# s22s/erased-cells

Measured on AMD Instinct MI355X. Metric: Gcells/s + HBM-GB/s roofline %, u8/u16->f64 16384^2, 1/2/4/8 GPUs, higher is better.
Workload: dtype f64

## Files before the change

erased-cells_amd/csrc/ec_binop_kernels.hpp:

```cpp
#pragma once

#include "ec_device.hpp"

namespace ecd {

constexpr int kBlock = 256;
constexpr int kWave = 64;
constexpr int kWavesPerBlock = kBlock / kWave;

template <bool NT, typename V>
__device__ __forceinline__ V load_vec(const V* p) {
    if constexpr (NT) return nt_load(p);
    else return plain_load(p);
}

__device__ __forceinline__ size_t two_front_tile() {
    const size_t b = blockIdx.x;
    return (b & 1) ? size_t(gridDim.x) - 1 - (b >> 1) : (b >> 1);
}

template <typename L, typename R, int OP, int U>
__device__ __forceinline__ void binop_direct_tile(const L* __restrict__ l, const R* __restrict__ r,
                                                  double* __restrict__ out, size_t npairs, size_t tile, unsigned cacheable) {
    using D2 = vec<double, 2>;
    constexpr bool FP = is_fp<L>::value || is_fp<R>::value;
    constexpr bool SM = is_small_int<L>::value && is_small_int<R>::value;
    constexpr size_t TILE = size_t(kBlock) * U;
    D2* __restrict__ op = reinterpret_cast<D2*>(out);
    const size_t base = tile * TILE + threadIdx.x;
    if (tile * TILE + TILE <= npairs) {
        cells<L, 2> a[U];
        cells<R, 2> b[U];
        policy_arms<2>(cacheable, [&](auto bits) {
            constexpr unsigned B = decltype(bits)::value;
#pragma unroll
            for (int j = 0; j < U; ++j) {
                a[j] = load_cells<!(B & 1u), L, 2>(l + 2 * (base + size_t(j) * kBlock));
                b[j] = load_cells<!(B & 2u), R, 2>(r + 2 * (base + size_t(j) * kBlock));
            }
        });
        if constexpr (OP == EC_DIV && SM && !FP) {
#pragma unroll
            for (int j = 0; j < U; ++j) {
                double av[2], bv[2], q[2], y[2], e[2];
                bool zero = false;
#pragma unroll
                for (int k = 0; k < 2; ++k) {
                    av[k] = to_f64(a[j][k]);
                    bv[k] = to_f64(b[j][k]);
                    zero = zero || b[j][k] == 0;
                }
                div_small_int_nonzero_staged<2>(av, bv, q, y, e);
                if (__builtin_expect(__builtin_amdgcn_ballot_w64(zero) != 0, 0)) {
#pragma unroll
                    for (int i = 0; i < 2; ++i) q[i] = bv[i] == 0.0 ? div_by_zero(av[i]) : q[i];
                }
                nt_store(D2{q[0], q[1]}, op + base + size_t(j) * kBlock);
            }
        } else {
#pragma unroll
            for (int j = 0; j < U; ++j) {
                const double av[2] = {to_f64(a[j][0]), to_f64(a[j][1])}, bv[2] = {to_f64(b[j][0]), to_f64(b[j][1])};
                double o[2];
                cell_op_n<OP, FP, SM, 2>(av, bv, o);
                nt_store(D2{o[0], o[1]}, op + base + size_t(j) * kBlock);
            }
        }
    } else {
#pragma unroll
        for (int j = 0; j < U; ++j) {
            const size_t p = base + size_t(j) * kBlock;
            if (p < npairs) {
                const cells<L, 2> a = load_cells<true, L, 2>(l + 2 * p);
                const cells<R, 2> b = load_cells<true, R, 2>(r + 2 * p);
                D2 o;
                o.x = cell_op<OP, FP, SM>(to_f64(a[0]), to_f64(b[0]));
                o.y = cell_op<OP, FP, SM>(to_f64(a[1]), to_f64(b[1]));
                nt_store(o, op + p);
            }
        }
    }
}

template <typename L, typename R, int OP, int U>
__device__ __forceinline__ void binop_direct_body(const L* __restrict__ l, const R* __restrict__ r,
                                                  double* __restrict__ out, size_t n, unsigned head_and_policy) {
    constexpr bool FP = is_fp<L>::value || is_fp<R>::value;
    constexpr bool SM = is_small_int<L>::value && is_small_int<R>::value;
    const unsigned head = head_and_policy & 0xffu, cacheable = head_and_policy >> 8;
    if (head) {
        if (blockIdx.x == 0 && threadIdx.x < head)
            st_cell(cell_op<OP, FP, SM>(to_f64(ld_cell(l + threadIdx.x)), to_f64(ld_cell(r + threadIdx.x))), out + threadIdx.x);
        l += head;
        r += head;
        out += head;
        n -= head;
    }
    binop_direct_tile<L, R, OP, U>(l, r, out, n >> 1, two_front_tile(), cacheable);
    if ((n & 1) && blockIdx.x == 0 && threadIdx.x == 0)
        st_cell(cell_op<OP, FP, SM>(to_f64(ld_cell(l + n - 1)), to_f64(ld_cell(r + n - 1))), out + n - 1);
}

template <typename L, int OP, int U, bool NANRULE = true>
__device__ __forceinline__ void binop_scalar_tile(const L* __restrict__ l, double s, double* __restrict__ out,
                                                  size_t npairs, size_t tile, unsigned cacheable) {
    using D2 = vec<double, 2>;
    constexpr bool FP = NANRULE;
    constexpr size_t TILE = size_t(kBlock) * U;
    D2* __restrict__ op = reinterpret_cast<D2*>(out);
    const size_t base = tile * TILE + threadIdx.x;
    if (tile * TILE + TILE <= npairs) {
        cells<L, 2> a[U];
        policy_arms<1>(cacheable, [&](auto bits) {
            constexpr unsigned B = decltype(bits)::value;
#pragma unroll
            for (int j = 0; j < U; ++j) a[j] = load_cells<!(B & 1u), L, 2>(l + 2 * (base + size_t(j) * kBlock));
        });
#pragma unroll
        for (int j = 0; j < U; ++j) {
            const double av[2] = {to_f64(a[j][0]), to_f64(a[j][1])}, bv[2] = {s, s};
            double o[2];
            cell_op_n<OP, FP, false, 2>(av, bv, o);
            nt_store(D2{o[0], o[1]}, op + base + size_t(j) * kBlock);
        }
    } else {
#pragma unroll
        for (int j = 0; j < U; ++j) {
            const size_t p = base + size_t(j) * kBlock;
            if (p < npairs) {
                const cells<L, 2> a = load_cells<true, L, 2>(l + 2 * p);
                D2 o;
                o.x = cell_op<OP, FP>(to_f64(a[0]), s);
                o.y = cell_op<OP, FP>(to_f64(a[1]), s);
                nt_store(o, op + p);
            }
        }
    }
}

template <typename L, int OP, int U, bool NANRULE = true>
__global__ __launch_bounds__(kBlock) void k_binop_scalar_direct(const L* __restrict__ l, double s,
                                                                double* __restrict__ out, size_t n, unsigned head_and_policy) {
    const unsigned head = head_and_policy & 0xffu, cacheable = head_and_policy >> 8;
    if (head) {
        if (blockIdx.x == 0 && threadIdx.x < head) st_cell(cell_op<OP, true>(to_f64(ld_cell(l + threadIdx.x)), s), out + threadIdx.x);
        l += head;
        out += head;
        n -= head;
    }
    binop_scalar_tile<L, OP, U, NANRULE>(l, s, out, n >> 1, two_front_tile(), cacheable);
    if ((n & 1) && blockIdx.x == 0 && threadIdx.x == 0) st_cell(cell_op<OP, true>(to_f64(ld_cell(l + n - 1)), s), out + n - 1);
}

template <typename L, typename R, int OP>
__global__ __launch_bounds__(kBlock) void k_binop_cellwise(const L* __restrict__ l, const R* __restrict__ r,
                                                           double* __restrict__ out, size_t n) {
    constexpr bool FP = is_fp<L>::value || is_fp<R>::value;
    constexpr bool SM = is_small_int<L>::value && is_small_int<R>::value;
    const size_t stride = size_t(gridDim.x) * kBlock;
    for (size_t i = size_t(blockIdx.x) * kBlock + threadIdx.x; i < n; i += stride)
        out[i] = cell_op<OP, FP, SM>(to_f64(l[i]), to_f64(r[i]));
}

template <typename L, int OP>
__global__ __launch_bounds__(kBlock) void k_binop_scalar_cellwise(const L* __restrict__ l, double s,
                                                                  double* __restrict__ out, size_t n) {
    const size_t stride = size_t(gridDim.x) * kBlock;
    for (size_t i = size_t(blockIdx.x) * kBlock + threadIdx.x; i < n; i += stride)
        out[i] = cell_op<OP, true>(to_f64(l[i]), s);
}

constexpr int kLdsChunks = 2;
constexpr size_t kLdsWaveCells = 128 * kLdsChunks;

template <typename T>
struct Staged {
    static constexpr bool value = sizeof(T) <= 4;
    using Load = vec<uint32_t, int(sizeof(T))>;
    static constexpr int kSlabBytes = value ? int(kLdsWaveCells * sizeof(T)) : 16;
};

using u32x4 = vec<uint32_t, 4>;

template <typename L, typename R, int OP>
__device__ __forceinline__ void binop_lds_body(const L* __restrict__ l, const R* __restrict__ r,
                                               double* __restrict__ out, size_t n) {
    using L2 = vec<L, 2>;
    using R2 = vec<R, 2>;
    using D2 = vec<double, 2>;
    constexpr bool FP = is_fp<L>::value || is_fp<R>::value;
    constexpr bool SM = is_small_int<L>::value && is_small_int<R>::value;
    constexpr bool SL = Staged<L>::value, SR = Staged<R>::value;

    __shared__ __attribute__((aligned(16))) unsigned char slab_l[kWavesPerBlock][Staged<L>::kSlabBytes];
    __shared__ __attribute__((aligned(16))) unsigned char slab_r[kWavesPerBlock][Staged<R>::kSlabBytes];

    const int lane = threadIdx.x & (kWave - 1);
    const int wave = threadIdx.x / kWave;
    const size_t nfull = n / kLdsWaveCells;
    const size_t t = two_front_tile() * kWavesPerBlock + wave;
    if (t < nfull) {
        const size_t cell0 = t * kLdsWaveCells;
        L2 a[kLdsChunks];
        R2 b[kLdsChunks];
        typename Staged<L>::Load sl{};
        typename Staged<R>::Load sr{};
        if constexpr (SL) {
            sl = nt_load(reinterpret_cast<const typename Staged<L>::Load*>(l + cell0) + lane);
        } else {
#pragma unroll
            for (int j = 0; j < kLdsChunks; ++j) a[j] = nt_load(reinterpret_cast<const L2*>(l + cell0) + j * kWave + lane);
        }
        if constexpr (SR) {
            sr = nt_load(reinterpret_cast<const typename Staged<R>::Load*>(r + cell0) + lane);
        } else {
#pragma unroll
            for (int j = 0; j < kLdsChunks; ++j) b[j] = nt_load(reinterpret_cast<const R2*>(r + cell0) + j * kWave + lane);
        }
        if constexpr (SL) reinterpret_cast<typename Staged<L>::Load*>(slab_l[wave])[lane] = sl;
        if constexpr (SR) reinterpret_cast<typename Staged<R>::Load*>(slab_r[wave])[lane] = sr;
        if constexpr (SL || SR) {
            __builtin_amdgcn_fence(__ATOMIC_RELEASE, "wavefront");
            __builtin_amdgcn_wave_barrier();
            __builtin_amdgcn_fence(__ATOMIC_ACQUIRE, "wavefront");
        }
        if constexpr (SL) {
#pragma unroll
            for (int j = 0; j < kLdsChunks; ++j) a[j] = reinterpret_cast<const L2*>(slab_l[wave])[j * kWave + lane];
        }
        if constexpr (SR) {
#pragma unroll
            for (int j = 0; j < kLdsChunks; ++j) b[j] = reinterpret_cast<const R2*>(slab_r[wave])[j * kWave + lane];
        }
        D2* o2 = reinterpret_cast<D2*>(out + cell0);
#pragma unroll
        for (int j = 0; j < kLdsChunks; ++j) {
            const double av[2] = {to_f64(a[j].x), to_f64(a[j].y)}, bv[2] = {to_f64(b[j].x), to_f64(b[j].y)};
            double o[2];
            cell_op_n<OP, FP, SM, 2>(av, bv, o);
            nt_store(D2{o[0], o[1]}, o2 + j * kWave + lane);
        }
    }
    if (blockIdx.x == 0)
        for (size_t i = nfull * kLdsWaveCells + threadIdx.x; i < n; i += kBlock)
            st_cell(cell_op<OP, FP, SM>(to_f64(ld_cell(l + i)), to_f64(ld_cell(r + i))), out + i);
}

template <typename L, typename R, int OP, int U>
__global__ __launch_bounds__(kBlock) void k_binop_direct(const L* __restrict__ l, const R* __restrict__ r,
                                                         double* __restrict__ out, size_t n, unsigned head = 0) {
    binop_direct_body<L, R, OP, U>(l, r, out, n, head);
}

template <typename L, typename R, int OP>
__global__ __launch_bounds__(kBlock) void k_binop_lds(const L* __restrict__ l, const R* __restrict__ r,
                                                      double* __restrict__ out, size_t n) {
    binop_lds_body<L, R, OP>(l, r, out, n);
}

__device__ __forceinline__ void mask_and_body(const uint8_t* __restrict__ lm, const uint8_t* __restrict__ rm,
                                              uint8_t* __restrict__ om, size_t n, unsigned cacheable) {
    const size_t ngroups = n / 16;
    const u32x4* __restrict__ a = reinterpret_cast<const u32x4*>(lm);
    const u32x4* __restrict__ b = reinterpret_cast<const u32x4*>(rm);
    u32x4* __restrict__ o = reinterpret_cast<u32x4*>(om);
    const size_t stride = size_t(gridDim.x) * kBlock;
    for (size_t g = size_t(blockIdx.x) * kBlock + threadIdx.x; g < ngroups; g += stride) {
        u32x4 x, y;
        policy_arms<2>(cacheable >> 2, [&](auto bits) {
            constexpr unsigned B = decltype(bits)::value;
            x = load_vec<!(B & 1u)>(a + g);
            y = load_vec<!(B & 2u)>(b + g);
        });
        mask_store(x & y, o + g);
    }
    if (blockIdx.x == 0)
        for (size_t i = ngroups * 16 + threadIdx.x; i < n; i += kBlock) st_cell<uint8_t>(ld_cell(lm + i) & ld_cell(rm + i), om + i);
}

template <typename L, typename R, int OP, int U, bool LDS>
__global__ __launch_bounds__(kBlock) void k_masked_binop(const L* __restrict__ l, const uint8_t* __restrict__ lm,
                                                         const R* __restrict__ r, const uint8_t* __restrict__ rm,
                                                         double* __restrict__ out, uint8_t* __restrict__ om, size_t n,
                                                         unsigned head) {
    if constexpr (LDS) binop_lds_body<L, R, OP>(l, r, out, n);
    else binop_direct_body<L, R, OP, U>(l, r, out, n, head);
    mask_and_body(lm, rm, om, n, head >> 8);
}

template <typename L, typename R, int OP>
__global__ __launch_bounds__(kBlock) void k_masked_binop_cellwise(const L* __restrict__ l, const uint8_t* __restrict__ lm,
                                                                  const R* __restrict__ r, const uint8_t* __restrict__ rm,
                                                                  double* __restrict__ out, uint8_t* __restrict__ om, size_t n) {
    constexpr bool FP = is_fp<L>::value || is_fp<R>::value;
    constexpr bool SM = is_small_int<L>::value && is_small_int<R>::value;
    const size_t stride = size_t(gridDim.x) * kBlock;
    for (size_t i = size_t(blockIdx.x) * kBlock + threadIdx.x; i < n; i += stride) {
        out[i] = cell_op<OP, FP, SM>(to_f64(l[i]), to_f64(r[i]));
        om[i] = lm[i] & rm[i];
    }
}

}
```

erased-cells_amd/csrc/ec_binop_tu.hpp:

```cpp
#pragma once

#include <hip/hip_runtime.h>

#include <cmath>

#include "ec_binop_kernels.hpp"
#include "ec_runtime.hpp"

namespace ecd {

static inline unsigned lds_cap(int knob, int rule_kb) { return static_cast<unsigned>(knob >= 0 ? knob : rule_kb) << 10; }

template <typename L, typename R, int OP>
static ec_status launch_binop_pair(const void* l, const void* r, size_t n, double* out, hipStream_t s) {
    const Tuning& tu = tuning();
    const L* lp = static_cast<const L*>(l);
    const R* rp = static_cast<const R*>(r);
    constexpr int U = kBinopU;
    if (!aligned16(l, r, out)) {
        k_binop_cellwise<L, R, OP><<<grid_capped((n + kBlock - 1) / kBlock, 8), kBlock, 0, s>>>(lp, rp, out, n);
        return check_launch("binop(cellwise)");
    }
    constexpr bool kCanStage = Staged<L>::value || Staged<R>::value;
    const int variant = tu.binop_variant.load();
    const size_t stream_bytes[2] = {n * sizeof(L), l == r ? 0 : n * sizeof(R)};
    unsigned policy = cache_plan(stream_bytes, 2, n * sizeof(double));
    if (l == r && (policy & 1u)) policy |= 2u;
    constexpr bool kRulePair = kCanStage && ((sizeof(L) == 8) != (sizeof(R) == 8)) && (sizeof(L) <= 4 || sizeof(R) <= 4);
    const bool by_rule = variant < 0 && kRulePair && policy == 0 && n >= (size_t(1) << 20);
    if (kCanStage && (variant == 1 || by_rule)) {
        const size_t tiles = (n / kLdsWaveCells + kWavesPerBlock - 1) / kWavesPerBlock;
        constexpr unsigned kStatic = kWavesPerBlock * unsigned(Staged<L>::kSlabBytes + Staged<R>::kSlabBytes);
        const int knob = tu.binop_lds_kb.load();
        const unsigned lds = knob >= 0 ? unsigned(knob) << 10 : by_rule ? 32000u - kStatic : 0u;
        k_binop_lds<L, R, OP><<<grid_for(tiles), kBlock, lds, s>>>(lp, rp, out, n);
        if (by_rule) lds_rule_launches().fetch_add(1, std::memory_order_relaxed);
        return check_launch(by_rule ? "binop(lds, by rule)" : "binop(lds)");
    }
    const LoadedStream st[2] = {{l, sizeof(L)}, {r, sizeof(R)}};
    const unsigned head = peel_head(st, 2, n);
    const size_t tiles = (((n - head) >> 1) + size_t(kBlock) * U - 1) / (size_t(kBlock) * U);
    k_binop_direct<L, R, OP, U><<<grid_for(tiles), kBlock, lds_cap(tuning().binop_lds_kb.load(), sizeof(L) == 8 && sizeof(R) == 8 ? 48 : 0), s>>>(lp, rp, out, n, head | (policy << 8));
    return check_launch("binop(direct)");
}

template <typename L, typename R, int OP>
static ec_status launch_masked_pair(const void* l, const uint8_t* lm, const void* r, const uint8_t* rm, size_t n,
                                    double* out, uint8_t* om, hipStream_t s) {
    const Tuning& tu = tuning();
    const L* lp = static_cast<const L*>(l);
    const R* rp = static_cast<const R*>(r);
    constexpr int U = kBinopU;
    if (!aligned16(l, r, out) || !aligned16(lm, rm, om)) {
        k_masked_binop_cellwise<L, R, OP><<<grid_capped((n + kBlock - 1) / kBlock, 8), kBlock, 0, s>>>(lp, lm, rp, rm, out, om, n);
        return check_launch("masked_binop(cellwise)");
    }
    constexpr bool kCanStage = Staged<L>::value || Staged<R>::value;
    if (kCanStage && tu.binop_variant == 1) {
        const size_t tiles = (n / kLdsWaveCells + kWavesPerBlock - 1) / kWavesPerBlock;
        k_masked_binop<L, R, OP, U, true><<<grid_for(tiles), kBlock, lds_cap(tu.binop_lds_kb.load(), 0), s>>>(lp, lm, rp, rm, out, om, n, 0u);
        return check_launch("masked_binop(lds)");
    }
    const LoadedStream st[2] = {{l, sizeof(L)}, {r, sizeof(R)}};
    const unsigned head = peel_head(st, 2, n);
    const size_t tiles = (((n - head) >> 1) + size_t(kBlock) * U - 1) / (size_t(kBlock) * U);
    const size_t stream_bytes[4] = {n * sizeof(L), l == r ? 0 : n * sizeof(R), n, lm == rm ? 0 : n};
    unsigned policy = cache_plan(stream_bytes, 4, n * sizeof(double));
    if (l == r && (policy & 1u)) policy |= 2u;
    if (lm == rm && (policy & 4u)) policy |= 8u;
    k_masked_binop<L, R, OP, U, false><<<grid_for(tiles), kBlock, 0, s>>>(lp, lm, rp, rm, out, om, n, head | (policy << 8));
    return check_launch("masked_binop(direct)");
}


template <typename L, int OP>
static ec_status launch_scalar(const void* l, double rhs, size_t n, double* out, hipStream_t s) {
    const L* lp = static_cast<const L*>(l);
    constexpr int U = kBinopU;
    if (!aligned16(l, out, out)) {
        k_binop_scalar_cellwise<L, OP><<<grid_capped((n + kBlock - 1) / kBlock, 8), kBlock, 0, s>>>(lp, rhs, out, n);
        return check_launch("binop_scalar(cellwise)");
    }
    const LoadedStream st[1] = {{l, sizeof(L)}};
    const unsigned head = peel_head(st, 1, n);
    const size_t tiles = (((n - head) >> 1) + size_t(kBlock) * U - 1) / (size_t(kBlock) * U);
    const size_t stream_bytes[1] = {n * sizeof(L)};
    const unsigned policy = cache_plan(stream_bytes, 1, n * sizeof(double));
    const unsigned lds = lds_cap(tuning().scalar_lds_kb.load(), sizeof(L) == 8 ? 32 : 0);
    if constexpr (!is_fp<L>::value) {
        if (std::isfinite(rhs) && !(OP == EC_DIV && rhs == 0.0)) {
            k_binop_scalar_direct<L, OP, U, false><<<grid_for(tiles), kBlock, lds, s>>>(lp, rhs, out, n, head | (policy << 8));
            return check_launch("binop_scalar(direct, no NaN possible)");
        }
    }
    k_binop_scalar_direct<L, OP, U><<<grid_for(tiles), kBlock, lds, s>>>(lp, rhs, out, n, head | (policy << 8));
    return check_launch("binop_scalar(direct)");
}

template <int OP>
ec_status dispatch_binop(int lt, const void* l, int rt, const void* r, size_t n, double* out, hipStream_t s) {
#define EC_ROW(LID, LT)                                                                         \
    case LID:                                                                                   \
        switch (rt) {                                                                           \
            case EC_U8: return launch_binop_pair<LT, uint8_t, OP>(l, r, n, out, s);             \
            case EC_U16: return launch_binop_pair<LT, uint16_t, OP>(l, r, n, out, s);           \
            case EC_U32: return launch_binop_pair<LT, uint32_t, OP>(l, r, n, out, s);           \
            case EC_U64: return launch_binop_pair<LT, uint64_t, OP>(l, r, n, out, s);           \
            case EC_I8: return launch_binop_pair<LT, int8_t, OP>(l, r, n, out, s);              \
            case EC_I16: return launch_binop_pair<LT, int16_t, OP>(l, r, n, out, s);            \
            case EC_I32: return launch_binop_pair<LT, int32_t, OP>(l, r, n, out, s);            \
            case EC_I64: return launch_binop_pair<LT, int64_t, OP>(l, r, n, out, s);            \
            case EC_F32: return launch_binop_pair<LT, float, OP>(l, r, n, out, s);              \
            case EC_F64: return launch_binop_pair<LT, double, OP>(l, r, n, out, s);             \
        }                                                                                       \
        break;
    switch (lt) { EC_WITH_CT(EC_ROW) }
#undef EC_ROW
    return set_error(EC_ERR_UNSUPPORTED_TYPE, "binop: bad dtype");
// ... 44 lines not shown
```

erased-cells_amd/csrc/ec_expr_jit.hip:

```cpp
#include <dlfcn.h>
#include <hip/hip_runtime.h>

#include <atomic>
#include <condition_variable>
#include <cstdlib>
#include <cstring>
#include <algorithm>
#include <deque>
#include <iterator>
#include <limits>
#include <map>
#include <memory>
#include <mutex>
#include <string>
#include <thread>
#include <unordered_map>
#include <vector>

#include "ec_expr_jit.hpp"
#include "ec_lattice.hpp"
#include "ec_runtime.hpp"

namespace ecd {

namespace {

const char* const kPrelude = R"SRC(
typedef double D2 __attribute__((ext_vector_type(2)));
typedef unsigned int U2 __attribute__((ext_vector_type(2)));
typedef unsigned int U4 __attribute__((ext_vector_type(4)));
typedef unsigned short W1 __attribute__((aligned(1)));
typedef unsigned int W2 __attribute__((aligned(1)));
typedef U2 W4 __attribute__((aligned(1)));
typedef U4 W8 __attribute__((aligned(1)));
typedef D2 DO __attribute__((aligned(1)));
typedef unsigned long long u64;
// the result's 16-byte store: write-through and non-temporal, as the library's own value stores (ec_device.hpp stream_store_asm;
// `s_nop 1`: a VALU write of the data registers needs two wait states behind a store of more than 64 bits)
static __device__ __forceinline__ void st16(D2 v, DO* p) { asm volatile("global_store_dwordx4 %0, %1, off sc1 nt\n\ts_nop 1" ::"v"(p), "v"(v)); }
#define FOR _Pragma("unroll") for (int i = 0; i < N; ++i)
// cv_bin_op! on NaN (ec_device.hpp cell_op<OP, true>): the first NaN operand, quieted; the x86 default NaN when neither is one
static __device__ __forceinline__ double fixnan(double t, double a, double b) {
    const u64 f = (a != a) ? (__builtin_bit_cast(u64, a) | 0x0008000000000000ull)
                : (b != b) ? (__builtin_bit_cast(u64, b) | 0x0008000000000000ull) : 0xFFF8000000000000ull;
    return (t != t) ? __builtin_bit_cast(double, f) : t;
}
// The quotient of two integers of magnitude ≤ 131070 held as f64 (≤ 16-bit cells, their sums and differences): v_rcp_f64, one
// Newton step, the quotient, its exact residual and one correction — ec_device.hpp div_small_int, proven against the IEEE
// expansion on that whole square (tools/div_small_check.hip); b == 0 gives what the f64 divide gives: ±inf, the x86 default
// NaN for 0/0 (an integer-derived zero is +0).
static __device__ __forceinline__ double divs(double a, double b) {
    double y = __builtin_amdgcn_rcp(b);
    const double e = __builtin_fma(-b, y, 1.0);
    y = __builtin_fma(y, e, y);
    double q = a * y;
    const double r = __builtin_fma(-b, q, a);
    q = __builtin_fma(r, y, q);
    const double z = a == 0.0 ? __builtin_bit_cast(double, 0xFFF8000000000000ull) : (a > 0.0 ? __builtin_inf() : -__builtin_inf());
    return b == 0.0 ? z : q;
}
// tested once per pair of cells (v_cmp_u_f64 r0, r1 is true when either is NaN), handled out of line, wave-uniform branch
#define NANFIX(A, B)                                                                                  \
    {                                                                                                 \
        bool nan = false;                                                                             \
        _Pragma("unroll") for (int i = 0; i + 1 < N; i += 2) nan = nan || __builtin_isunordered(t[i], t[i + 1]); \
        if (N & 1) nan = nan || (t[N - 1] != t[N - 1]);                                               \
        if (__builtin_expect(__builtin_amdgcn_ballot_w64(nan) != 0, 0)) { FOR t[i] = fixnan(t[i], A, B); } \
    }
)SRC";

const char* const kCellType[10] = {"unsigned char", "unsigned short", "unsigned int", "unsigned long long", "signed char",
                                   "short",         "int",            "long long",    "float",              "double"};

// ... 124 lines not shown
             "        if (__builtin_amdgcn_ballot_w64(special) == 0) {\n"
             "            _Pragma(\"unroll\") for (int i = 0; i < NC; ++i) {\n"
             "                fmin = __builtin_fmin(fmin, valid[i] ? o[i] : fmin);\n                fmax = __builtin_fmax(fmax, valid[i] ? o[i] : fmax);\n            }\n"
             "        } else {\n"
             "            _Pragma(\"unroll\") for (int i = 0; i < NC; ++i)\n                if (valid[i]) {\n"
             "                    const long long k = okey(o[i]);\n                    a = ~k > a ? ~k : a;\n                    b = k > b ? k : b;\n                }\n"
             "        }\n"
             "    }\n"
             "    {\n        const long long k0 = okey(fmin), k1 = okey(fmax);\n        a = ~k0 > a ? ~k0 : a;\n        b = k1 > b ? k1 : b;\n    }\n"
             "    if (blockIdx.x == 0 && threadIdx.x < 2) {  // the peeled head cell (lane 0) and the odd tail cell (lane 1)\n"
             "        const bool do_it = threadIdx.x == 0 ? head != 0 : ((n - head) & 1) != 0;\n"
             "        const unsigned long i = threadIdx.x == 0 ? 0 : n - 1;\n"
             "        if (do_it) {\n";
        for (int k2 = 0; k2 < 4; ++k2) {
            const std::string K = std::to_string(k2);
            o += "            const double a" + K + "[1] = {" + (k2 < ns ? "cell" + K + "(p" + K + ", i)" : std::string("0.0")) + "};\n";
        }
        o += "            double q[1];\n            run<1>(a0, a1, a2, a3, c0, c1, c2, c3, c4, c5, c6, c7, q);\n            bool ok = true;\n";
        for (int k2 = 0; k2 < ea.nmask; ++k2)
            o += "            ok = ok && __builtin_nontemporal_load((const unsigned char*)m" + std::to_string(k2) + " + i) != 0;\n";
        o += "            if (ok) {\n                const long long k = okey(q[0]);\n                a = ~k > a ? ~k : a;\n                b = k > b ? k : b;\n            }\n"
             "        }\n    }\n"
             "    __shared__ long long sa[256], sb[256];\n"
             "    sa[threadIdx.x] = a;\n    sb[threadIdx.x] = b;\n    __syncthreads();\n"
             "    for (int w = 128; w > 0; w >>= 1) {\n"
             "        if ((int)threadIdx.x < w) {\n"
             "            sa[threadIdx.x] = sa[threadIdx.x + w] > sa[threadIdx.x] ? sa[threadIdx.x + w] : sa[threadIdx.x];\n"
             "            sb[threadIdx.x] = sb[threadIdx.x + w] > sb[threadIdx.x] ? sb[threadIdx.x + w] : sb[threadIdx.x];\n"
             "        }\n        __syncthreads();\n    }\n"
             "    if (threadIdx.x == 0) {\n"
             "        __hip_atomic_fetch_max(keys2, sa[0], __ATOMIC_RELAXED, __HIP_MEMORY_SCOPE_AGENT);\n"
             "        __hip_atomic_fetch_max(keys2 + 1, sb[0], __ATOMIC_RELAXED, __HIP_MEMORY_SCOPE_AGENT);\n"
             "    }\n}\n";
        return o;
    }
    o += "extern \"C\" __global__ __launch_bounds__(256) void ec_expr_jit(const char* p0, const char* p1, const char* p2, const char* p3, ";
    o += scal;
    o += ", double* __restrict__ out, unsigned long n, unsigned head, const char* m0, const char* m1, const char* m2, const char* m3, "
         "unsigned char* __restrict__ out_mask) {\n"
         "    constexpr int U = 2, NC = 2 * U;\n"
         "    const unsigned long npairs = (n - head) >> 1, TILE = 256ul * U;\n"
         "    const unsigned long blk = blockIdx.x, tile = (blk & 1) ? (unsigned long)gridDim.x - 1 - (blk >> 1) : (blk >> 1);  // two fronts\n"
         "    const unsigned long base = tile * TILE + threadIdx.x;\n"
         "    DO* op = (DO*)(out + head);\n"
         "    double s0[NC] = {}, s1[NC] = {}, s2[NC] = {}, s3[NC] = {}, o[NC];\n";
    for (int k = 0; k < ns; ++k)
        o += "    const char* b" + std::to_string(k) + " = p" + std::to_string(k) + " + (unsigned long)head * " + std::to_string(ecl::size_of(ea.dt[k])) + ";\n";
    o += "    const bool full = tile * TILE + TILE <= npairs;\n"
         "    if (full) {\n        _Pragma(\"unroll\") for (int j = 0; j < U; ++j) {\n            const unsigned long pr = base + j * 256ul;\n";
    for (int k = 0; k < ns; ++k) {
        const std::string K = std::to_string(k);
        o += "            ld" + K + "(b" + K + ", pr, s" + K + "[2 * j], s" + K + "[2 * j + 1]);\n";
    }
    o += "        }\n    } else {\n        _Pragma(\"unroll\") for (int j = 0; j < U; ++j) {\n            const unsigned long pr = base + j * 256ul;\n            if (pr < npairs) {\n";
    for (int k = 0; k < ns; ++k) {
        const std::string K = std::to_string(k);
        o += "                ld" + K + "(b" + K + ", pr, s" + K + "[2 * j], s" + K + "[2 * j + 1]);\n";
    }
    o += "            }\n        }\n    }\n"
         "    run<NC>(s0, s1, s2, s3, c0, c1, c2, c3, c4, c5, c6, c7, o);\n"
         "    _Pragma(\"unroll\") for (int j = 0; j < U; ++j) {\n        const unsigned long pr = base + j * 256ul;\n"
         "        if (full || pr < npairs) st16(D2{o[2 * j], o[2 * j + 1]}, op + pr);\n    }\n"
         "    if (blockIdx.x == 0 && threadIdx.x < 2) {  // the peeled head cell (lane 0) and the odd tail cell (lane 1)\n"
         "        const bool do_it = threadIdx.x == 0 ? head != 0 : ((n - head) & 1) != 0;\n"
         "        const unsigned long i = threadIdx.x == 0 ? 0 : n - 1;\n"
         "        if (do_it) {\n";
    for (int k = 0; k < 4; ++k) {
        const std::string K = std::to_string(k);
        o += "            const double a" + K + "[1] = {" + (k < ns ? "cell" + K + "(p" + K + ", i)" : std::string("0.0")) + "};\n";
    }
    o += "            double q[1];\n            run<1>(a0, a1, a2, a3, c0, c1, c2, c3, c4, c5, c6, c7, q);\n"
         "            __builtin_nontemporal_store(q[0], out + i);\n        }\n    }\n";
    if (ea.nmask > 0) {
        o += "    {\n        const unsigned long ngroups = n / 16, stride = (unsigned long)gridDim.x * 256ul;\n"
             "        for (unsigned long g = (unsigned long)blockIdx.x * 256ul + threadIdx.x; g < ngroups; g += stride) {\n"
             "            U4 acc = {0xffffffffu, 0xffffffffu, 0xffffffffu, 0xffffffffu};\n";
        for (int k = 0; k < ea.nmask; ++k) {
            const bool nt = !((ea.cacheable >> (4 + k)) & 1u);
            o += std::string("            acc &= ") + (nt ? "__builtin_nontemporal_load(" : "*(") + "(const W8*)m" + std::to_string(k) + " + g);\n";
        }
        o += "            __builtin_nontemporal_store(acc, (W8*)out_mask + g);\n        }\n"
             "        if (blockIdx.x == 0)\n            for (unsigned long i = ngroups * 16 + threadIdx.x; i < n; i += 256ul) {\n"
             "                unsigned char acc = __builtin_nontemporal_load((const unsigned char*)m0 + i);\n";
        for (int k = 1; k < ea.nmask; ++k)
            o += "                acc &= __builtin_nontemporal_load((const unsigned char*)m" + std::to_string(k) + " + i);\n";
        o += "                __builtin_nontemporal_store(acc, out_mask + i);\n            }\n    }\n";
    }
    o += "}\n";
    return o;
}

namespace {

struct Hiprtc {
    int (*create)(void** prog, const char* src, const char* name, int nh, const char** headers, const char** names) = nullptr;
    int (*compile)(void* prog, int nopt, const char** opts) = nullptr;
    int (*code_size)(void* prog, size_t* n) = nullptr;
    int (*code)(void* prog, char* out) = nullptr;
    int (*log_size)(void* prog, size_t* n) = nullptr;
    int (*log)(void* prog, char* out) = nullptr;
    int (*destroy)(void** prog) = nullptr;
    const char* (*error_string)(int) = nullptr;
    std::string load_error;
};

Hiprtc g_rtc;
std::once_flag g_rtc_once;

void load_hiprtc() {
    void* h = nullptr;
    if (const char* named = std::getenv("EC_HIPRTC_LIB")) {
        h = dlopen(named, RTLD_NOW | RTLD_LOCAL);
    } else {
        for (const char* name : {"libhiprtc.so", "libhiprtc.so.7", "libhiprtc.so.6"})
            if ((h = dlopen(name, RTLD_NOW | RTLD_LOCAL)) != nullptr) break;
    }
    if (!h) {
        const char* e = dlerror();
        g_rtc.load_error = std::string("libhiprtc not found: ") + (e ? e : "dlopen failed");
        return;
    }
#define EC_SYM(field, name) g_rtc.field = reinterpret_cast<decltype(g_rtc.field)>(dlsym(h, name))
    EC_SYM(create, "hiprtcCreateProgram");
    EC_SYM(compile, "hiprtcCompileProgram");
    EC_SYM(code_size, "hiprtcGetCodeSize");
    EC_SYM(code, "hiprtcGetCode");
    EC_SYM(log_size, "hiprtcGetProgramLogSize");
    EC_SYM(log, "hiprtcGetProgramLog");
    EC_SYM(destroy, "hiprtcDestroyProgram");
    EC_SYM(error_string, "hiprtcGetErrorString");
#undef EC_SYM
    if (!g_rtc.create || !g_rtc.compile || !g_rtc.code_size || !g_rtc.code || !g_rtc.destroy) g_rtc.load_error = "libhiprtc lacks an expected symbol";
}

const Hiprtc* hiprtc() {
    std::call_once(g_rtc_once, load_hiprtc);
    return g_rtc.load_error.empty() ? &g_rtc : nullptr;
}

// ... 177 lines not shown
                std::lock_guard<std::mutex> lk(g_mu);
                g_compiler.ensure();
                g_queue.push_back(e);
                g_cv.notify_one();
            }
            return EC_OK;
        } else {
            return EC_OK;
        }
    }
    if (state != kReady) return EC_OK;
    hipFunction_t fn = nullptr;
    {
        std::lock_guard<std::mutex> lk(e->mu);
        auto it = e->fn.find(dev);
        if (it == e->fn.end()) {
            hipStreamCaptureStatus cap = hipStreamCaptureStatusNone;
            if (s && hipStreamIsCapturing(s, &cap) == hipSuccess && cap != hipStreamCaptureStatusNone) return EC_OK;
            hipModule_t mod = nullptr;
            st = check_hip(hipModuleLoadData(&mod, e->code.data()), "hipModuleLoadData(expression kernel)");
            if (st != EC_OK) return st;
            st = check_hip(hipModuleGetFunction(&fn, mod, "ec_expr_jit"), "hipModuleGetFunction(ec_expr_jit)");
            if (st != EC_OK) {
                (void)hipModuleUnload(mod);
                return st;
            }
            e->modules.emplace_back(dev, mod);
            e->fn.emplace(dev, fn);
        } else {
            fn = it->second;
        }
    }
    const char* p[4] = {static_cast<const char*>(ea.p[0]), static_cast<const char*>(ea.p[1]), static_cast<const char*>(ea.p[2]),
                        static_cast<const char*>(ea.p[3])};
    double c[8];
    for (int k = 0; k < 8; ++k) c[k] = ea.sc[k];
    unsigned long nn = n;
    unsigned head = ea.head;
    const char* m[4] = {reinterpret_cast<const char*>(ea.m[0]), reinterpret_cast<const char*>(ea.m[1]), reinterpret_cast<const char*>(ea.m[2]),
                        reinterpret_cast<const char*>(ea.m[3])};
    const size_t npairs = (n - head) >> 1;
    if (reduce) {
        long long a0k = ~order_key<double>(std::numeric_limits<double>::max()), b0k = order_key<double>(std::numeric_limits<double>::lowest());
        long long* k2 = reinterpret_cast<long long*>(keys2);
        void* params[] = {&p[0], &p[1], &p[2], &p[3], &c[0], &c[1], &c[2], &c[3], &c[4], &c[5], &c[6], &c[7], &k2, &nn, &head,
                          &m[0], &m[1], &m[2], &m[3], &a0k, &b0k};
        const size_t per_tile = size_t(256) * reduce_u();
        const size_t tiles = (npairs + per_tile - 1) / per_tile;
        const unsigned grid = static_cast<unsigned>(std::min<size_t>(std::max<size_t>(tiles, 1), size_t(device_cus()) * 8));
        st = check_hip(hipModuleLaunchKernel(fn, grid, 1, 1, 256, 1, 1, 0, s, params, nullptr), "hipModuleLaunchKernel(ec_expr_jit, reduce)");
    } else {
        void* params[] = {&p[0], &p[1], &p[2], &p[3], &c[0], &c[1], &c[2], &c[3], &c[4], &c[5], &c[6], &c[7], &out, &nn, &head,
                          &m[0], &m[1], &m[2], &m[3], &out_mask};
        const unsigned grid = grid_for((npairs + 511) / 512);
        st = check_hip(hipModuleLaunchKernel(fn, grid, 1, 1, 256, 1, 1, 0, s, params, nullptr), "hipModuleLaunchKernel(ec_expr_jit)");
    }
    if (st != EC_OK) return st;
    g_jit_launches.fetch_add(1, std::memory_order_relaxed);
    *launched = true;
    return EC_OK;
}

void expr_jit_release() {
    g_compiler.stop();
    std::vector<std::shared_ptr<Entry>> all;
    {
        std::lock_guard<std::mutex> lk(g_mu);
        for (auto& kv : g_cache) all.push_back(kv.second);
    }
    for (auto& e : all) {
        std::lock_guard<std::mutex> lk(e->mu);
        for (auto& dm : e->modules)
            if (hipSetDevice(dm.first) == hipSuccess) (void)hipModuleUnload(dm.second);
        e->modules.clear();
        e->fn.clear();
    }
}

int64_t expr_jit_stat(const char* key, bool* known) {
    *known = true;
    if (!std::strcmp(key, "expr_jit_compiles")) return g_compiles.load(std::memory_order_relaxed);
    if (!std::strcmp(key, "expr_jit_failures")) return g_failures.load(std::memory_order_relaxed);
    if (!std::strcmp(key, "expr_jit_launches")) return g_jit_launches.load(std::memory_order_relaxed);
    if (!std::strcmp(key, "expr_jit_programs")) {
        std::lock_guard<std::mutex> lk(g_mu);
        return static_cast<int64_t>(g_cache.size());
    }
    *known = false;
    return 0;
}

}
```

erased-cells_amd/csrc/ec_stream_tile.hpp:

```cpp
#pragma once

#include "ec_binop_kernels.hpp"
#include "ec_runtime.hpp"

namespace ecd {

using D2 = vec<double, 2>;

struct no_stream {};
template <int C> struct raw_pair;
template <> struct raw_pair<0> { using type = no_stream; };
template <> struct raw_pair<1> { using type = uint16_t; };
template <> struct raw_pair<2> { using type = uint32_t; };
template <> struct raw_pair<4> { using type = vec<uint32_t, 2>; };
template <> struct raw_pair<8> { using type = vec<uint32_t, 4>; };

template <bool NT, typename A>
__device__ __forceinline__ uint8_t mask_and_cell(const A& a, size_t i) {
    if constexpr (NT) {
        uint8_t acc = ld_cell(a.m[0] + i);
        for (int k = 1; k < a.nmask; ++k) acc &= ld_cell(a.m[k] + i);
        return acc;
    } else {
        uint8_t acc = a.m[0][i];
        for (int k = 1; k < a.nmask; ++k) acc &= a.m[k][i];
        return acc;
    }
}

template <typename A>
__device__ __forceinline__ void mask_phase(const A& a, uint8_t* __restrict__ out_mask, size_t n) {
    if (a.nmask > 0) {
        const size_t ngroups = n / 16;
        const size_t stride = size_t(gridDim.x) * kBlock;
        u32x4* __restrict__ om = reinterpret_cast<u32x4*>(out_mask);
        for (size_t g = size_t(blockIdx.x) * kBlock + threadIdx.x; g < ngroups; g += stride) {
            u32x4 acc = {0xffffffffu, 0xffffffffu, 0xffffffffu, 0xffffffffu};
            for (int k = 0; k < a.nmask; ++k) {
                const u32x4* mk = reinterpret_cast<const u32x4*>(a.m[k]) + g;
                u32x4 x;
                policy_arms<1>(a.cacheable >> (4 + k), [&](auto bits) { x = load_vec<!(decltype(bits)::value & 1u)>(mk); });
                acc &= x;
            }
            mask_store(acc, om + g);
        }
        if (blockIdx.x == 0)
            for (size_t i = ngroups * 16 + threadIdx.x; i < n; i += kBlock) st_cell(mask_and_cell<true>(a, i), out_mask + i);
    }
}

template <int U, int NP, int C0, int C1, int C2, int C3, typename A, typename Body, typename OneCell>
__device__ __forceinline__ void stream_tile(const A& a, const void* const (&p)[4], unsigned policy, Body&& body, OneCell&& one_cell,
                                            double* __restrict__ out, uint8_t* __restrict__ out_mask, size_t n) {
    static_assert(U % NP == 0, "chunks of the tile");
    using R0 = typename raw_pair<C0>::type;
    using R1 = typename raw_pair<C1>::type;
    using R2 = typename raw_pair<C2>::type;
    using R3 = typename raw_pair<C3>::type;
    const unsigned head = a.head;
    const size_t npairs = (n - head) >> 1;
    constexpr size_t TILE = size_t(kBlock) * U;
    const size_t tile = two_front_tile();
    const size_t base = tile * TILE + threadIdx.x;
    const bool full = tile * TILE + TILE <= npairs;
    D2* __restrict__ op = reinterpret_cast<D2*>(out + head);
    const R0* b0 = reinterpret_cast<const R0*>(static_cast<const char*>(p[0]) + size_t(head) * C0);
    const R1* b1 = reinterpret_cast<const R1*>(static_cast<const char*>(p[1]) + size_t(head) * C1);
    const R2* b2 = reinterpret_cast<const R2*>(static_cast<const char*>(p[2]) + size_t(head) * C2);
    const R3* b3 = reinterpret_cast<const R3*>(static_cast<const char*>(p[3]) + size_t(head) * C3);

    R0 q0[U] = {};
    R1 q1[U] = {};
    R2 q2[U] = {};
    R3 q3[U] = {};
    if (full) {
        constexpr int kStreams = (C0 != 0) + (C1 != 0) + (C2 != 0) + (C3 != 0);
        constexpr int kBit1 = (C0 != 0), kBit2 = kBit1 + (C1 != 0), kBit3 = kBit2 + (C2 != 0);
        policy_arms<kStreams>(policy, [&](auto bits) {
            constexpr unsigned B = decltype(bits)::value;
#pragma unroll
            for (int j = 0; j < U; ++j) {
                const size_t pr = base + size_t(j) * kBlock;
                if constexpr (C0 != 0) q0[j] = load_vec<!(B & 1u)>(b0 + pr);
                if constexpr (C1 != 0) q1[j] = load_vec<!((B >> kBit1) & 1u)>(b1 + pr);
                if constexpr (C2 != 0) q2[j] = load_vec<!((B >> kBit2) & 1u)>(b2 + pr);
                if constexpr (C3 != 0) q3[j] = load_vec<!((B >> kBit3) & 1u)>(b3 + pr);
            }
        });
    } else {
#pragma unroll
        for (int j = 0; j < U; ++j) {
            const size_t pr = base + size_t(j) * kBlock;
            if (pr < npairs) {
                if constexpr (C0 != 0) q0[j] = nt_load(b0 + pr);
                if constexpr (C1 != 0) q1[j] = nt_load(b1 + pr);
                if constexpr (C2 != 0) q2[j] = nt_load(b2 + pr);
                if constexpr (C3 != 0) q3[j] = nt_load(b3 + pr);
            }
        }
    }
#pragma unroll
    for (int c = 0; c < U; c += NP) {
        R0 r0[NP];
        R1 r1[NP];
        R2 r2[NP];
        R3 r3[NP];
#pragma unroll
        for (int j = 0; j < NP; ++j) {
            r0[j] = q0[c + j];
            r1[j] = q1[c + j];
            r2[j] = q2[c + j];
            r3[j] = q3[c + j];
        }
        double o[2 * NP];
        body(std::integral_constant<int, NP>{}, r0, r1, r2, r3, o);
#pragma unroll
        for (int j = 0; j < NP; ++j) {
            const size_t pr = base + size_t(c + j) * kBlock;
            if (full || pr < npairs) nt_store(D2{o[2 * j], o[2 * j + 1]}, op + pr);
        }
    }
    if (blockIdx.x == 0 && threadIdx.x < 2) {
        const bool do_it = threadIdx.x == 0 ? head != 0 : ((n - head) & 1) != 0;
        const size_t i = threadIdx.x == 0 ? 0 : n - 1;
        if (do_it) st_cell(one_cell(i), out + i);
    }
    mask_phase(a, out_mask, n);
}

template <int U, typename... KArgs, typename... Args>
void launch_stream_tile(void (*kern)(KArgs...), unsigned head, size_t n, hipStream_t s, const Args&... args) {
    const size_t per_tile = size_t(kBlock) * U;
    const unsigned grid = grid_for((((n - head) >> 1) + per_tile - 1) / per_tile);
    hipLaunchKernelGGL(kern, dim3(grid), dim3(kBlock), static_cast<unsigned>(tuning().fused_lds_kb.load()) << 10, s, args...);
}

}
```

Before: 597.2.

## Tile-align mask AND with value tiles instead of separate grid-stride pass

```diff
diff --git a/erased-cells_amd/csrc/ec_binop_kernels.hpp b/erased-cells_amd/csrc/ec_binop_kernels.hpp
--- a/erased-cells_amd/csrc/ec_binop_kernels.hpp
+++ b/erased-cells_amd/csrc/ec_binop_kernels.hpp
@@ -1,6 +1,7 @@
 #pragma once
 
 #include "ec_device.hpp"
+#include "ec_mask_tile.hpp"
 
 namespace ecd {
 
@@ -19,9 +20,71 @@
     return (b & 1) ? size_t(gridDim.x) - 1 - (b >> 1) : (b >> 1);
 }
 
-template <typename L, typename R, int OP, int U>
+using u32x4 = vec<uint32_t, 4>;
+
+struct NoTileMasks {
+    __device__ __forceinline__ void words(size_t) {}
+};
+
+template <int NM, int CELLS>
+struct TileMasks {
+    static_assert(CELLS % 16 == 0 && CELLS / 16 <= 256, "one 16-byte word per lane");
+    const uint8_t* m[NM];
+    uint8_t* out;
+    int nmask;
+    unsigned policy;
+    size_t n;
+
+    template <typename P>
+    __device__ __forceinline__ TileMasks(const P (&masks)[NM], uint8_t* out_mask, int count, unsigned policy_bits, size_t cells)
+        : out(out_mask), nmask(count), policy(policy_bits), n(cells) {
+#pragma unroll
+        for (int k = 0; k < NM; ++k) m[k] = k < count ? masks[k] : masks[0];
+    }
+
+    typedef const __attribute__((address_space(1))) typename under_aligned<u32x4>::type* global_word;
+    __device__ __forceinline__ void words(size_t tile) {
+        if (nmask > 0 && threadIdx.x < CELLS / 16) {
+            const size_t at = tile * CELLS + 16 * threadIdx.x;
+            uint64_t from[NM];
+#pragma unroll
+            for (int k = 0; k < NM; ++k) {
+                from[k] = reinterpret_cast<uint64_t>(m[k] + at);
+                asm volatile("" : "+v"(from[k]));
+            }
+            u32x4 w[NM];
+            policy_arms<NM>(policy, [&](auto bits) { load_words<decltype(bits)::value>(w, from); });
+            u32x4 acc = w[0];
+#pragma unroll
+            for (int k = 1; k < NM; ++k) acc &= w[k];
+            mask_store(acc, reinterpret_cast<u32x4*>(out + at));
+        }
+    }
+    template <unsigned B, int K = 0>
+    __device__ __forceinline__ void load_words(u32x4 (&w)[NM], const uint64_t (&from)[NM]) {
+        if constexpr (K < NM) {
+            if constexpr ((B >> K) & 1u) w[K] = *reinterpret_cast<global_word>(from[K]);
+            else w[K] = __builtin_nontemporal_load(reinterpret_cast<global_word>(from[K]));
+            load_words<B, K + 1>(w, from);
+        }
+    }
+    __device__ __forceinline__ void rest(size_t tile, bool words_done) {
+        if (nmask > 0) {
+            const MaskRange r = mask_tile_range(tile, gridDim.x, n, CELLS);
+            for (size_t i = r.begin + (words_done ? size_t(CELLS) : 0) + threadIdx.x; i < r.end; i += 256) {
+                uint8_t acc = ld_cell(m[0] + i);
+#pragma unroll
+                for (int k = 1; k < NM; ++k)
+                    if (k < nmask) acc &= ld_cell(m[k] + i);
+                st_cell(acc, out + i);
+            }
+        }
+    }
+};
+
+template <typename L, typename R, int OP, int U, typename Masks>
 __device__ __forceinline__ void binop_direct_tile(const L* __restrict__ l, const R* __restrict__ r,
-                                                  double* __restrict__ out, size_t npairs, size_t tile, unsigned cacheable) {
+                                                  double* __restrict__ out, size_t npairs, size_t tile, unsigned cacheable, Masks& masks) {
     using D2 = vec<double, 2>;
     constexpr bool FP = is_fp<L>::value || is_fp<R>::value;
     constexpr bool SM = is_small_int<L>::value && is_small_int<R>::value;
@@ -39,6 +102,7 @@
                 b[j] = load_cells<!(B & 2u), R, 2>(r + 2 * (base + size_t(j) * kBlock));
             }
         });
+        masks.words(tile);
         if constexpr (OP == EC_DIV && SM && !FP) {
 #pragma unroll
             for (int j = 0; j < U; ++j) {
@@ -82,9 +146,9 @@
     }
 }
 
-template <typename L, typename R, int OP, int U>
+template <typename L, typename R, int OP, int U, typename Masks>
 __device__ __forceinline__ void binop_direct_body(const L* __restrict__ l, const R* __restrict__ r,
-                                                  double* __restrict__ out, size_t n, unsigned head_and_policy) {
+                                                  double* __restrict__ out, size_t n, unsigned head_and_policy, Masks& masks) {
     constexpr bool FP = is_fp<L>::value || is_fp<R>::value;
     constexpr bool SM = is_small_int<L>::value && is_small_int<R>::value;
     const unsigned head = head_and_policy & 0xffu, cacheable = head_and_policy >> 8;
@@ -96,7 +160,7 @@
         out += head;
         n -= head;
     }
-    binop_direct_tile<L, R, OP, U>(l, r, out, n >> 1, two_front_tile(), cacheable);
+    binop_direct_tile<L, R, OP, U>(l, r, out, n >> 1, two_front_tile(), cacheable, masks);
     if ((n & 1) && blockIdx.x == 0 && threadIdx.x == 0)
         st_cell(cell_op<OP, FP, SM>(to_f64(ld_cell(l + n - 1)), to_f64(ld_cell(r + n - 1))), out + n - 1);
 }
@@ -180,11 +244,9 @@
     static constexpr int kSlabBytes = value ? int(kLdsWaveCells * sizeof(T)) : 16;
 };
 
-using u32x4 = vec<uint32_t, 4>;
-
-template <typename L, typename R, int OP>
+template <typename L, typename R, int OP, typename Masks>
 __device__ __forceinline__ void binop_lds_body(const L* __restrict__ l, const R* __restrict__ r,
-                                               double* __restrict__ out, size_t n) {
+                                               double* __restrict__ out, size_t n, Masks& masks) {
     using L2 = vec<L, 2>;
     using R2 = vec<R, 2>;
     using D2 = vec<double, 2>;
@@ -198,7 +260,9 @@
     const int lane = threadIdx.x & (kWave - 1);
     const int wave = threadIdx.x / kWave;
     const size_t nfull = n / kLdsWaveCells;
-    const size_t t = two_front_tile() * kWavesPerBlock + wave;
+    const size_t tile = two_front_tile();
+    const size_t t = tile * kWavesPerBlock + wave;
+    const bool mask_words = mask_tile_whole(tile, n, kWavesPerBlock * kLdsWaveCells);
     if (t < nfull) {
         const size_t cell0 = t * kLdsWaveCells;
         L2 a[kLdsChunks];
@@ -217,6 +281,7 @@
 #pragma unroll
             for (int j = 0; j < kLdsChunks; ++j) b[j] = nt_load(reinterpret_cast<const R2*>(r + cell0) + j * kWave + lane);
         }
+        if (mask_words) masks.words(tile);
         if constexpr (SL) reinterpret_cast<typename Staged<L>::Load*>(slab_l[wave])[lane] = sl;
         if constexpr (SR) reinterpret_cast<typename Staged<R>::Load*>(slab_r[wave])[lane] = sr;
         if constexpr (SL || SR) {
@@ -249,33 +314,15 @@
 template <typename L, typename R, int OP, int U>
 __global__ __launch_bounds__(kBlock) void k_binop_direct(const L* __restrict__ l, const R* __restrict__ r,
                                                          double* __restrict__ out, size_t n, unsigned head = 0) {
-    binop_direct_body<L, R, OP, U>(l, r, out, n, head);
+    NoTileMasks none;
+    binop_direct_body<L, R, OP, U>(l, r, out, n, head, none);
 }
 
 template <typename L, typename R, int OP>
 __global__ __launch_bounds__(kBlock) void k_binop_lds(const L* __restrict__ l, const R* __restrict__ r,
                                                       double* __restrict__ out, size_t n) {
-    binop_lds_body<L, R, OP>(l, r, out, n);
-}
-
-__device__ __forceinline__ void mask_and_body(const uint8_t* __restrict__ lm, const uint8_t* __restrict__ rm,
-                                              uint8_t* __restrict__ om, size_t n, unsigned cacheable) {
-    const size_t ngroups = n / 16;
-    const u32x4* __restrict__ a = reinterpret_cast<const u32x4*>(lm);
-    const u32x4* __restrict__ b = reinterpret_cast<const u32x4*>(rm);
-    u32x4* __restrict__ o = reinterpret_cast<u32x4*>(om);
-    const size_t stride = size_t(gridDim.x) * kBlock;
-    for (size_t g = size_t(blockIdx.x) * kBlock + threadIdx.x; g < ngroups; g += stride) {
-        u32x4 x, y;
-        policy_arms<2>(cacheable >> 2, [&](auto bits) {
-            constexpr unsigned B = decltype(bits)::value;
-            x = load_vec<!(B & 1u)>(a + g);
-            y = load_vec<!(B & 2u)>(b + g);
-        });
-        mask_store(x & y, o + g);
-    }
-    if (blockIdx.x == 0)
-        for (size_t i = ngroups * 16 + threadIdx.x; i < n; i += kBlock) st_cell<uint8_t>(ld_cell(lm + i) & ld_cell(rm + i), om + i);
+    NoTileMasks none;
+    binop_lds_body<L, R, OP>(l, r, out, n, none);
 }
 
 template <typename L, typename R, int OP, int U, bool LDS>
@@ -283,9 +330,19 @@
                                                          const R* __restrict__ r, const uint8_t* __restrict__ rm,
                                                          double* __restrict__ out, uint8_t* __restrict__ om, size_t n,
                                                          unsigned head) {
-    if constexpr (LDS) binop_lds_body<L, R, OP>(l, r, out, n);
-    else binop_direct_body<L, R, OP, U>(l, r, out, n, head);
-    mask_and_body(lm, rm, om, n, head >> 8);
+    constexpr int CELLS = LDS ? int(kWavesPerBlock * kLdsWaveCells) : 2 * kBlock * U;
+    const uint8_t* const both[2] = {lm, rm};
+    TileMasks<2, CELLS> masks(both, om, 2, head >> 10, n);
+    const size_t tile = two_front_tile();
+    bool words_done;
+    if constexpr (LDS) {
+        binop_lds_body<L, R, OP>(l, r, out, n, masks);
+        words_done = mask_tile_whole(tile, n, CELLS);
+    } else {
+        binop_direct_body<L, R, OP, U>(l, r, out, n, head, masks);
+        words_done = (tile + 1) * (size_t(kBlock) * U) <= ((n - (head & 0xffu)) >> 1);
+    }
+    masks.rest(tile, words_done);
 }
 
 template <typename L, typename R, int OP>
diff --git a/erased-cells_amd/csrc/ec_binop_tu.hpp b/erased-cells_amd/csrc/ec_binop_tu.hpp
--- a/erased-cells_amd/csrc/ec_binop_tu.hpp
+++ b/erased-cells_amd/csrc/ec_binop_tu.hpp
@@ -63,7 +63,7 @@
     }
     const LoadedStream st[2] = {{l, sizeof(L)}, {r, sizeof(R)}};
     const unsigned head = peel_head(st, 2, n);
-    const size_t tiles = (((n - head) >> 1) + size_t(kBlock) * U - 1) / (size_t(kBlock) * U);
+    const size_t tiles = pair_grid_tiles(n, head, size_t(2) * kBlock * U);
     const size_t stream_bytes[4] = {n * sizeof(L), l == r ? 0 : n * sizeof(R), n, lm == rm ? 0 : n};
     unsigned policy = cache_plan(stream_bytes, 4, n * sizeof(double));
     if (l == r && (policy & 1u)) policy |= 2u;
diff --git a/erased-cells_amd/csrc/ec_expr_jit.hip b/erased-cells_amd/csrc/ec_expr_jit.hip
--- a/erased-cells_amd/csrc/ec_expr_jit.hip
+++ b/erased-cells_amd/csrc/ec_expr_jit.hip
@@ -19,6 +19,7 @@
 
 #include "ec_expr_jit.hpp"
 #include "ec_lattice.hpp"
+#include "ec_mask_tile.hpp"
 #include "ec_runtime.hpp"
 
 namespace ecd {
@@ -249,14 +250,26 @@
         const std::string K = std::to_string(k);
         o += "            ld" + K + "(b" + K + ", pr, s" + K + "[2 * j], s" + K + "[2 * j + 1]);\n";
     }
-    o += "        }\n    } else {\n        _Pragma(\"unroll\") for (int j = 0; j < U; ++j) {\n            const unsigned long pr = base + j * 256ul;\n            if (pr < npairs) {\n";
+    o += "        }\n";
+    if (ea.nmask > 0) {
+        o += "        if (threadIdx.x < 64) {\n";
+        std::string all;
+        for (int k = 0; k < ea.nmask; ++k) {
+            const bool nt = !((ea.cacheable >> (4 + k)) & 1u);
+            const std::string K = std::to_string(k);
+            o += "            const U4 mw" + K + " = " + (nt ? "__builtin_nontemporal_load(" : "*(") + "(const W8*)(m" + K + " + tile * 1024ul) + threadIdx.x);\n";
+            all += (k ? " & mw" : "mw") + K;
+        }
+        o += "            __builtin_nontemporal_store(" + all + ", (W8*)(out_mask + tile * 1024ul) + threadIdx.x);\n        }\n";
+    }
+    o += "    } else {\n        _Pragma(\"unroll\") for (int j = 0; j < U; ++j) {\n            const unsigned long pr = base + j * 256ul;\n            if (pr < npairs) {\n";
     for (int k = 0; k < ns; ++k) {
         const std::string K = std::to_string(k);
         o += "                ld" + K + "(b" + K + ", pr, s" + K + "[2 * j], s" + K + "[2 * j + 1]);\n";
     }
     o += "            }\n        }\n    }\n"
-         "    run<NC>(s0, s1, s2, s3, c0, c1, c2, c3, c4, c5, c6, c7, o);\n"
-         "    _Pragma(\"unroll\") for (int j = 0; j < U; ++j) {\n        const unsigned long pr = base + j * 256ul;\n"
+         "    run<NC>(s0, s1, s2, s3, c0, c1, c2, c3, c4, c5, c6, c7, o);\n";
+    o += "    _Pragma(\"unroll\") for (int j = 0; j < U; ++j) {\n        const unsigned long pr = base + j * 256ul;\n"
          "        if (full || pr < npairs) st16(D2{o[2 * j], o[2 * j + 1]}, op + pr);\n    }\n"
          "    if (blockIdx.x == 0 && threadIdx.x < 2) {  // the peeled head cell (lane 0) and the odd tail cell (lane 1)\n"
          "        const bool do_it = threadIdx.x == 0 ? head != 0 : ((n - head) & 1) != 0;\n"
@@ -269,19 +282,13 @@
     o += "            double q[1];\n            run<1>(a0, a1, a2, a3, c0, c1, c2, c3, c4, c5, c6, c7, q);\n"
          "            __builtin_nontemporal_store(q[0], out + i);\n        }\n    }\n";
     if (ea.nmask > 0) {
-        o += "    {\n        const unsigned long ngroups = n / 16, stride = (unsigned long)gridDim.x * 256ul;\n"
-             "        for (unsigned long g = (unsigned long)blockIdx.x * 256ul + threadIdx.x; g < ngroups; g += stride) {\n"
-             "            U4 acc = {0xffffffffu, 0xffffffffu, 0xffffffffu, 0xffffffffu};\n";
-        for (int k = 0; k < ea.nmask; ++k) {
-            const bool nt = !((ea.cacheable >> (4 + k)) & 1u);
-            o += std::string("            acc &= ") + (nt ? "__builtin_nontemporal_load(" : "*(") + "(const W8*)m" + std::to_string(k) + " + g);\n";
-        }
-        o += "            __builtin_nontemporal_store(acc, (W8*)out_mask + g);\n        }\n"
-             "        if (blockIdx.x == 0)\n            for (unsigned long i = ngroups * 16 + threadIdx.x; i < n; i += 256ul) {\n"
-             "                unsigned char acc = __builtin_nontemporal_load((const unsigned char*)m0 + i);\n";
+        o += "    {\n        const unsigned long lo = tile * 1024ul, hi = lo + 1024ul;\n"
+             "        const unsigned long rb = lo < n ? lo : n, re = (tile + 1 == gridDim.x || hi > n) ? n : hi;\n"
+             "        for (unsigned long i = rb + (full ? 1024ul : 0ul) + threadIdx.x; i < re; i += 256ul) {\n"
+             "            unsigned char acc = __builtin_nontemporal_load((const unsigned char*)m0 + i);\n";
         for (int k = 1; k < ea.nmask; ++k)
-            o += "                acc &= __builtin_nontemporal_load((const unsigned char*)m" + std::to_string(k) + " + i);\n";
-        o += "                __builtin_nontemporal_store(acc, out_mask + i);\n            }\n    }\n";
+            o += "            acc &= __builtin_nontemporal_load((const unsigned char*)m" + std::to_string(k) + " + i);\n";
+        o += "            __builtin_nontemporal_store(acc, out_mask + i);\n        }\n    }\n";
     }
     o += "}\n";
     return o;
@@ -565,7 +572,7 @@
     } else {
         void* params[] = {&p[0], &p[1], &p[2], &p[3], &c[0], &c[1], &c[2], &c[3], &c[4], &c[5], &c[6], &c[7], &out, &nn, &head,
                           &m[0], &m[1], &m[2], &m[3], &out_mask};
-        const unsigned grid = grid_for((npairs + 511) / 512);
+        const unsigned grid = grid_for(pair_grid_tiles(n, head, 1024));
         st = check_hip(hipModuleLaunchKernel(fn, grid, 1, 1, 256, 1, 1, 0, s, params, nullptr), "hipModuleLaunchKernel(ec_expr_jit)");
     }
     if (st != EC_OK) return st;
diff --git a/erased-cells_amd/csrc/ec_mask_tile.hpp b/erased-cells_amd/csrc/ec_mask_tile.hpp
--- /dev/null
+++ b/erased-cells_amd/csrc/ec_mask_tile.hpp
@@ -0,0 +1,32 @@
+#pragma once
+
+#include <stddef.h>
+
+#if defined(__HIPCC__) || defined(__CUDACC__)
+#define EC_MASK_TILE_FN __host__ __device__ inline
+#else
+#define EC_MASK_TILE_FN inline
+#endif
+
+namespace ecd {
+
+EC_MASK_TILE_FN size_t pair_grid_tiles(size_t n, unsigned head, size_t cells_per_tile) {
+    const size_t npairs = (n - head) >> 1, per_tile = cells_per_tile >> 1;
+    const size_t tiles = (npairs + per_tile - 1) / per_tile;
+    return tiles < 1 ? 1 : tiles;
+}
+
+struct MaskRange {
+    size_t begin, end;
+};
+
+EC_MASK_TILE_FN MaskRange mask_tile_range(size_t t, size_t grid, size_t n, size_t cells_per_tile) {
+    const size_t lo = t * cells_per_tile, hi = lo + cells_per_tile;
+    MaskRange r;
+    r.begin = lo < n ? lo : n;
+    r.end = (t + 1 == grid || hi > n) ? n : hi;
+    return r;
+}
+EC_MASK_TILE_FN bool mask_tile_whole(size_t t, size_t n, size_t cells_per_tile) { return (t + 1) * cells_per_tile <= n; }
+
+}
diff --git a/erased-cells_amd/csrc/ec_stream_tile.hpp b/erased-cells_amd/csrc/ec_stream_tile.hpp
--- a/erased-cells_amd/csrc/ec_stream_tile.hpp
+++ b/erased-cells_amd/csrc/ec_stream_tile.hpp
@@ -28,27 +28,6 @@
     }
 }
 
-template <typename A>
-__device__ __forceinline__ void mask_phase(const A& a, uint8_t* __restrict__ out_mask, size_t n) {
-    if (a.nmask > 0) {
-        const size_t ngroups = n / 16;
-        const size_t stride = size_t(gridDim.x) * kBlock;
-        u32x4* __restrict__ om = reinterpret_cast<u32x4*>(out_mask);
-        for (size_t g = size_t(blockIdx.x) * kBlock + threadIdx.x; g < ngroups; g += stride) {
-            u32x4 acc = {0xffffffffu, 0xffffffffu, 0xffffffffu, 0xffffffffu};
-            for (int k = 0; k < a.nmask; ++k) {
-                const u32x4* mk = reinterpret_cast<const u32x4*>(a.m[k]) + g;
-                u32x4 x;
-                policy_arms<1>(a.cacheable >> (4 + k), [&](auto bits) { x = load_vec<!(decltype(bits)::value & 1u)>(mk); });
-                acc &= x;
-            }
-            mask_store(acc, om + g);
-        }
-        if (blockIdx.x == 0)
-            for (size_t i = ngroups * 16 + threadIdx.x; i < n; i += kBlock) st_cell(mask_and_cell<true>(a, i), out_mask + i);
-    }
-}
-
 template <int U, int NP, int C0, int C1, int C2, int C3, typename A, typename Body, typename OneCell>
 __device__ __forceinline__ void stream_tile(const A& a, const void* const (&p)[4], unsigned policy, Body&& body, OneCell&& one_cell,
                                             double* __restrict__ out, uint8_t* __restrict__ out_mask, size_t n) {
@@ -69,6 +48,8 @@
     const R2* b2 = reinterpret_cast<const R2*>(static_cast<const char*>(p[2]) + size_t(head) * C2);
     const R3* b3 = reinterpret_cast<const R3*>(static_cast<const char*>(p[3]) + size_t(head) * C3);
 
+    TileMasks<4, int(2 * TILE)> masks(a.m, out_mask, a.nmask, unsigned(a.cacheable) >> 4, n);
+
     R0 q0[U] = {};
     R1 q1[U] = {};
     R2 q2[U] = {};
@@ -87,6 +68,7 @@
                 if constexpr (C3 != 0) q3[j] = load_vec<!((B >> kBit3) & 1u)>(b3 + pr);
             }
         });
+        masks.words(tile);
     } else {
 #pragma unroll
         for (int j = 0; j < U; ++j) {
@@ -125,13 +107,12 @@
         const size_t i = threadIdx.x == 0 ? 0 : n - 1;
         if (do_it) st_cell(one_cell(i), out + i);
     }
-    mask_phase(a, out_mask, n);
+    masks.rest(tile, full);
 }
 
 template <int U, typename... KArgs, typename... Args>
 void launch_stream_tile(void (*kern)(KArgs...), unsigned head, size_t n, hipStream_t s, const Args&... args) {
-    const size_t per_tile = size_t(kBlock) * U;
-    const unsigned grid = grid_for((((n - head) >> 1) + per_tile - 1) / per_tile);
+    const unsigned grid = grid_for(pair_grid_tiles(n, head, size_t(2) * kBlock * U));
     hipLaunchKernelGGL(kern, dim3(grid), dim3(kBlock), static_cast<unsigned>(tuning().fused_lds_kb.load()) << 10, s, args...);
 }
 
```

New measurement: 600.3 (median of 5 runs). Within noise of the previous version (+0.5%).
